# dhansmair/flamingo-mini

Measured on AMD Instinct MI355X. Metric: images/sec (fwd+bwd) flamingo-mini bs=32, higher is better.
Workload: dtype bf16

## Files before the change

flamingo-mini_amd/csrc/ff_api.hip:

```cpp
#include <stdarg.h>
#include <stdio.h>
#include <math.h>
#include <stdlib.h>
#include "ff_common.h"
#include "ff_internal.h"

namespace ff {

static thread_local char g_err[512] = "";
void set_error(const char* fmt, ...) {
    va_list ap;
    va_start(ap, fmt);
    vsnprintf(g_err, sizeof(g_err), fmt, ap);
    va_end(ap);
}
#ifdef FF_DEBUG
int dbg_switch(const char* name, int dflt) {
    const char* e = getenv(name);
    return e ? atoi(e) : dflt;
}
#endif
int check_launch(const char* what) {
    hipError_t e = hipGetLastError();
    if (e != hipSuccess) {
// ... 464 lines not shown
    return align_up(a.used);
}
struct XaScratch {
    void *dy1, *dH, *dxn, *dO, *dQs, *dKV, *dyn, *ws;
    size_t ws_bytes;
    float* lnx;
};
struct XaStash {
    void *dy1, *dH, *dQs;
    float *lnp_f = nullptr, *lnp_a = nullptr;
};
static bool xa_ln_deferrable(const XaDims& s) {
    static const int on = dbg_switch("FF_DEFER_LN", 1);
    return on != 0 && layernorm_bwd_deferrable(s.dt, s.d);
}
static size_t xa_stash_layout(const XaDims& s, void* base, size_t cap, XaStash& o) {
    Arena a(base, cap);
    const size_t M = (size_t)s.b * s.L;
    o.dy1 = a.take(M * s.d * s.es);
    o.dH = a.take(M * s.ffi * s.es);
    o.dQs = a.take(M * s.inner * s.es);
    if (xa_ln_deferrable(s)) {
        o.lnp_f = a.take<float>(layernorm_bwd_partial_bytes((int)M, s.d));
        o.lnp_a = a.take<float>(layernorm_bwd_partial_bytes((int)M, s.d));
    }
    return align_up(a.used);
}
static size_t xa_ws_bytes(const XaDims& s) {
    const int M = s.b * s.L, Mk = s.b * s.Nk;
    size_t w = 0;
    auto g = [&](int m, int n, int k) { w = std::max(w, gemm_workspace_bytes(s.dt, m, n, k, 1, 0)); };
    g(M, s.inner, s.d); g(Mk, 2 * s.inner, s.dv); g(M, s.d, s.inner); g(M, s.ffi, s.d); g(M, s.d, s.ffi);
    g(s.d, s.ffi, M); g(s.ffi, s.d, M); g(s.d, s.inner, M); g(s.inner, s.d, M); g(2 * s.inner, s.dv, Mk); g(Mk, s.dv, 2 * s.inner);
    w = std::max(w, layernorm_bwd_workspace(M, s.d));
    w = std::max(w, gate_grad_workspace(M, s.d));
    if (decode_ffw_supported(s.dt, M, s.d, s.ffi)) w = std::max(w, decode_ffw_workspace_bytes(s.d, s.ffi));
    return align_up(w) + align_up((size_t)s.b * s.H * s.L * 4);
}
// ... 32 lines not shown
    a.q = sq; a.o = sq; a.dq = sq; a.dout = sq;
    a.k = cached ? x.cached_k : sk;
    a.v = cached ? x.cached_v : sk;
    a.dk = sk; a.dv = sk;
    return a;
}

static bool xa_fused_enabled() {
    static const int v = dbg_switch("FF_XATTN_FUSED", 1);
    return v != 0;
}
static bool xa_ln3_enabled() {
    static const int v = dbg_switch("FF_XATTN_LN3", 1);
    return v != 0;
}
static XaFusedArgs xa_fused_args(const ff_xattn_desc& x, const XaDims& s, bool ext_kv) {
    XaFusedArgs a = {};
    a.batch = s.b; a.heads = s.H; a.n_q = s.L; a.n_kv = s.Nk; a.n_visual = s.nv; a.tt_stride = x.tt_stride; a.tt_offset = x.tt_offset;
    a.dim = s.d; a.inner = s.inner; a.scale = s.scale; a.eps = 1e-5f;
    static const int xcd_split = dbg_switch("FF_XATTN_XCD_SPLIT", 0);
    a.xcd_split = xcd_split;
    const ff_strides sk = {(long long)s.Nk * 2 * s.inner, 2LL * s.inner, s.dh};
    a.k = ext_kv ? x.cached_k : sk;
    a.v = ext_kv ? x.cached_v : sk;
    a.dk = sk; a.dv = sk;
    return a;
}

static bool xa_ln3_in_bwd(const ff_xattn_desc& x, const XaDims& s) {
    if (!xa_ln3_enabled() || !xa_fused_enabled() || !xa_fused_supported(s.dt, s.dh, s.d, s.inner) || x.sync == nullptr) return false;
    const XaFusedArgs fa = xa_fused_args(x, s, s.ext_kv);
    const int M = s.b * s.L;
    return xa_out_fusable(fa, s.dt, s.dh) && s.b <= layernorm_bwd_partial_blocks(M) && (size_t)s.b * (2 * (size_t)s.d + 2) * sizeof(float) <= layernorm_bwd_workspace(M, s.d);
}
static int xattn_fwd(const ff_xattn_desc* d, const void* y, const void* vf, const int* tt, const void* const* P, const void* ck,
                     const void* cv, void* y_out, void* saved, size_t saved_bytes, void* scratch, size_t scratch_bytes, hipStream_t st) {
    FF_TRY(xa_check(d));
    const bool cached = ck != nullptr;
    FF_CHECK(y && tt && P && y_out && saved && scratch && (cached ? cv != nullptr : vf != nullptr), FF_ERR_SHAPE, "xattn_fwd: null argument");
    const XaDims s(*d);
    FF_CHECK(s.ext_kv == cached, FF_ERR_SHAPE, "xattn_fwd: external K / V need their strides in the descriptor (cached_k / cached_v) and vice versa");
    XaSaved S;
    XaScratch W;
    FF_CHECK(xa_saved_layout(s, saved, saved_bytes, S) <= saved_bytes, FF_ERR_WORKSPACE, "xattn_fwd: saved buffer too small");
    FF_CHECK(xa_scratch_layout(s, scratch, scratch_bytes, false, W) <= scratch_bytes, FF_ERR_WORKSPACE, "xattn_fwd: scratch too small");
    const int M = s.b * s.L, Mk = s.b * s.Nk;
    const RowMap pd = plain_rows(s.d), pI = plain_rows(s.inner), pF = plain_rows(s.ffi), pV = plain_rows(s.dv), pKV = plain_rows(2 * s.inner);
    const void *Kp, *Vp;
    if (!cached) {
// ... 32 lines not shown
                     const void* saved, size_t saved_bytes, void* const* G, void* dy, void* dvf, void* scratch, size_t scratch_bytes,
                     hipStream_t st, const void* ext_k = nullptr, const void* ext_v = nullptr, void* dkv_out = nullptr,
                     void* stash = nullptr, size_t stash_bytes = 0) {
    FF_TRY(xa_check(d));
    const bool hoisted = ext_k != nullptr;
    FF_CHECK(y && tt && P && dy2 && saved && G && dy && scratch && (hoisted ? (ext_v && dkv_out) : vf != nullptr), FF_ERR_SHAPE,
             "xattn_bwd: null argument");
    const XaDims s(*d);
    FF_CHECK(s.ext_kv == hoisted, FF_ERR_SHAPE, "xattn_bwd: external K / V need their strides in the descriptor (cached_k / cached_v) and vice versa");
    XaSaved S;
    XaScratch W;
    FF_CHECK(xa_saved_layout(s, (void*)saved, saved_bytes, S) <= saved_bytes, FF_ERR_WORKSPACE, "xattn_bwd: saved buffer too small");
    FF_CHECK(xa_scratch_layout(s, scratch, scratch_bytes, true, W) <= scratch_bytes, FF_ERR_WORKSPACE, "xattn_bwd: scratch too small");
    XaStash T{W.dy1, W.dH, W.dQs};
    const bool defer = stash != nullptr;
    if (defer) FF_CHECK(xa_stash_layout(s, stash, stash_bytes, T) <= stash_bytes, FF_ERR_WORKSPACE, "xattn_bwd: stash too small");
    const bool defer_ln = defer && xa_ln_deferrable(s);
    if (defer_ln)
        FF_CHECK(((uintptr_t)y | (uintptr_t)dy | (uintptr_t)dy2 | (uintptr_t)P[2] | (uintptr_t)P[7]) % 16 == 0, FF_ERR_SHAPE,
                 "xattn_bwd (deferred weight gradients): y, d y_out, d y and the LayerNorm weights must be 16-byte aligned");
    LnPending pend_f, pend_a;
    const int M = s.b * s.L, Mk = s.b * s.Nk;
    const RowMap pd = plain_rows(s.d), pI = plain_rows(s.inner), pF = plain_rows(s.ffi), pV = plain_rows(s.dv), pKV = plain_rows(2 * s.inner);
    const size_t attn_ws_bytes = align_up((size_t)s.b * s.H * s.L * 4);
    const size_t gws = W.ws_bytes - attn_ws_bytes;
    float* attn_ws = (float*)((char*)W.ws + gws);

    if (!defer) FF_TRY(Gemm(s.dt, s.d, s.ffi, M).a(1, pd).b(1, pF).c(pF).problem(dy2, S.Aact, G[10], nullptr, nullptr, nullptr, P[1]).run(W.ws, gws, st));
    FF_TRY(Gemm(s.dt, M, s.ffi, s.d).a(0, pd).b(1, pF).c(pF).act_bwd(s.act).problem(dy2, P[10], T.dH, nullptr, S.Hpre, nullptr, P[1]).run(W.ws, gws, st));
    if (!defer) FF_TRY(Gemm(s.dt, s.ffi, s.d, M).a(1, pF).b(1, pd).c(pd).problem(T.dH, S.xn_f, G[9]).run(W.ws, gws, st));
    static const int fold_reduce = dbg_switch("FF_FOLD_SPLITK_LN", 1);
    int dxn_splits = 1;
    FF_TRY(Gemm(s.dt, M, s.d, s.ffi).a(0, pF).b(1, pd).c(pd).problem(T.dH, P[9], W.dxn).run(W.ws, gws, st, defer_ln && fold_reduce ? &dxn_splits : nullptr));
    {
        LnDots dots;
        dots.a = S.ffw_out; dots.alpha_a = P[1]; dots.out_a = G[1];
        dots.b = S.attn_out; dots.alpha_b = P[0]; dots.out_b = G[0];
        if (defer_ln) {
            LnArgs la = ln_args(s.dt, M, s.d, pd, pd, pd);
            if (dxn_splits > 1) { la.dy_splits = dxn_splits; la.dy_slab = (long long)M * s.d; }
            FF_TRY(layernorm_bwd(la, dxn_splits > 1 ? W.ws : W.dxn, S.y1, nullptr, P[7], S.mean_f, S.rstd_f, T.dy1, dy2, G[7], G[8], T.lnp_f,
                                 layernorm_bwd_partial_bytes(M, s.d), st, &dots, &pend_f));
            FF_CHECK(pend_f.partial, FF_ERR_SHAPE, "xattn_bwd: the one-pass LayerNorm backward did not apply in the deferred mode");
        } else FF_TRY(layernorm_bwd(ln_args(s.dt, M, s.d, pd, pd, pd), W.dxn, S.y1, nullptr, P[7], S.mean_f, S.rstd_f, T.dy1, dy2, G[7], G[8], W.ws, gws, st, &dots));
    }
    if (!defer) FF_TRY(Gemm(s.dt, s.d, s.inner, M).a(1, pd).b(1, pI).c(pI).problem(T.dy1, S.O, G[6], nullptr, nullptr, nullptr, P[0]).run(W.ws, gws, st));
    char* dK = hoisted ? (char*)dkv_out : (char*)W.dKV;
    char* dV = dK + (size_t)s.inner * s.es;
    const void* Kp = hoisted ? ext_k : S.KV;
    const void* Vp = hoisted ? ext_v : (const void*)((const char*)S.KV + (size_t)s.inner * s.es);
    bool dyn_fused = false, lnb_fused = false;
    float* lnb_partial = nullptr;
    if (xa_fused_enabled() && xa_fused_supported(s.dt, s.dh, s.d, s.inner)) {
        int single = 0;
        const XaFusedArgs fa = xa_fused_args(*d, s, hoisted);
        XaOutArgs oa = {(const bf16*)P[4], nullptr, (bf16*)W.dyn, nullptr, (unsigned*)d->sync};
        dyn_fused = d->sync != nullptr && xa_out_fusable(fa, s.dt, s.dh);
        if (dyn_fused && xa_ln3_in_bwd(*d, s)) {
            lnb_fused = true;
            lnb_partial = defer_ln ? T.lnp_a : (float*)W.ws;
            oa.out = nullptr;
            oa.ln_g = (const bf16*)P[2]; oa.ln_x = (const bf16*)y; oa.ln_res = (const bf16*)T.dy1; oa.ln_out = (bf16*)dy;
            oa.ln_mean = S.mean_a; oa.ln_rstd = S.rstd_a; oa.ln_part = W.lnx; oa.ln_wpart = lnb_partial;
        }
        FF_TRY(xa_dattn_bwd(fa, s.dt, s.dh, T.dy1, P[6], P[0], S.Qs, Kp, Vp, tt, S.O, S.lse, W.dO, T.dQs, dK, dV, attn_ws, &single, st,
                            dyn_fused ? &oa : nullptr));
        if (!single) FF_TRY(attention_bwd_dkv(xa_attn_desc(*d, s, hoisted), S.Qs, Kp, Vp, tt, W.dO, S.lse, attn_ws, dK, dV, st));
        if (lnb_fused && !defer_ln) {
            LnPending q;
            q.partial = lnb_partial; q.nblk = s.b; q.cols = s.d; q.dgamma = G[2]; q.dbeta = G[3];
            FF_TRY(layernorm_bwd_finish(s.dt, &q, 1, st));
        }
    } else {
        FF_TRY(Gemm(s.dt, M, s.inner, s.d).a(0, pd).b(1, pI).c(pI).problem(T.dy1, P[6], W.dO, nullptr, nullptr, nullptr, P[0]).run(W.ws, gws, st));
        FF_TRY(attention_bwd(xa_attn_desc(*d, s, hoisted), S.Qs, Kp, Vp, tt, S.O, W.dO, S.lse, T.dQs, dK, dV, attn_ws, (size_t)s.b * s.H * s.L * 4, st));
    }
    if (!defer) FF_TRY(Gemm(s.dt, s.inner, s.d, M).a(1, pI).b(1, pd).c(pd).scale(s.scale).problem(T.dQs, S.yn, G[4]).run(W.ws, gws, st));
    if (!hoisted) {
        FF_TRY(Gemm(s.dt, 2 * s.inner, s.dv, Mk).a(1, pKV).b(1, pV).c(pV).problem(W.dKV, vf, G[5]).run(W.ws, gws, st));
        if (dvf) FF_TRY(Gemm(s.dt, Mk, s.dv, 2 * s.inner).a(0, pKV).b(1, pV).c(pV).problem(W.dKV, P[5], dvf).run(W.ws, gws, st));
    }
// ... 26 lines not shown
    const int M = s.b * s.L;
    const RowMap pd = plain_rows(s.d), pI = plain_rows(s.inner), pF = plain_rows(s.ffi);
    LnPending ln_sets[2 * kGemmMaxZ];
    const bool finish_ln = xa_ln_deferrable(s);
    const int ln_blocks = layernorm_bwd_partial_blocks(M);
    Gemm g3(s.dt, s.d, s.ffi, M), g1(s.dt, s.ffi, s.d, M), go(s.dt, s.d, s.inner, M), gq(s.dt, s.inner, s.d, M);
    g3.a(1, pd).b(1, pF).c(pF);
    g1.a(1, pF).b(1, pd).c(pd);
    go.a(1, pd).b(1, pI).c(pI);
    gq.a(1, pI).b(1, pd).c(pd).scale(s.scale);
    for (int i = 0; i < n; i++) {
        XaSaved S;
        XaStash T;
        FF_CHECK(dy2[i] && saved[i] && stash[i], FF_ERR_SHAPE, "xattn_wgrad_grouped: null buffer of block %d", i);
        FF_CHECK(xa_saved_layout(s, (void*)saved[i], saved_bytes, S) <= saved_bytes, FF_ERR_WORKSPACE, "xattn_wgrad_grouped: saved buffer too small");
        FF_CHECK(xa_stash_layout(s, (void*)stash[i], stash_bytes, T) <= stash_bytes, FF_ERR_WORKSPACE, "xattn_wgrad_grouped: stash too small");
        const void* const* P = params + (size_t)i * FF_XATTN_PARAMS;
        void* const* G = grads + (size_t)i * FF_XATTN_PARAMS;
        FF_CHECK(G[10] && G[9] && G[6] && G[4] && P[0] && P[1], FF_ERR_SHAPE, "xattn_wgrad_grouped: null parameter / gradient of block %d", i);
        g3.problem(dy2[i], S.Aact, G[10], nullptr, nullptr, nullptr, P[1]);
        g1.problem(T.dH, S.xn_f, G[9]);
        go.problem(T.dy1, S.O, G[6], nullptr, nullptr, nullptr, P[0]);
        gq.problem(T.dQs, S.yn, G[4]);
        if (finish_ln) {
            FF_CHECK(G[0] && G[1] && G[2] && G[3] && G[7] && G[8], FF_ERR_SHAPE, "xattn_wgrad_grouped: null LayerNorm / gate gradient of block %d", i);
            LnPending& f = ln_sets[2 * i];
            f.partial = T.lnp_f; f.nblk = ln_blocks; f.cols = s.d; f.dgamma = G[7]; f.dbeta = G[8];
            f.alpha_a = P[1]; f.out_a = G[1]; f.alpha_b = P[0]; f.out_b = G[0];
            LnPending& q = ln_sets[2 * i + 1];
            q.partial = T.lnp_a; q.nblk = xa_ln3_in_bwd(*d, s) ? s.b : ln_blocks; q.cols = s.d; q.dgamma = G[2]; q.dbeta = G[3];
        }
    }
    if (finish_ln) FF_TRY(layernorm_bwd_finish(s.dt, ln_sets, 2 * n, st));
    FF_TRY(g3.run(ws, ws_bytes, st));
    FF_TRY(g1.run(ws, ws_bytes, st));
    FF_TRY(go.run(ws, ws_bytes, st));
    return gq.run(ws, ws_bytes, st);
}

static int kvp_check(const ff_kvproj_desc* d) {
    FF_CHECK(d, FF_ERR_SHAPE, "kv_project: null descriptor");
    FF_CHECK(d->dtype == FF_DTYPE_F32 || d->dtype == FF_DTYPE_BF16, FF_ERR_UNSUPPORTED, "kv_project: dtype %d", d->dtype);
// ... 171 lines not shown
    return ff::xattn_bwd(d, y, visual_features, text_time, params, dy_out, saved, saved_bytes, grads, dy, dvisual_features, scratch,
                         scratch_bytes, (hipStream_t)stream);
}

extern "C" int ff_xattn_block_bwd_kv(const ff_xattn_desc* d, const void* y, const void* k, const void* v, const int* text_time,
                                     const void* const* params, const void* dy_out, const void* saved, size_t saved_bytes,
                                     void* const* grads, void* dy, void* dkv, void* scratch, size_t scratch_bytes, ff_stream_t stream) {
    using namespace ff;
    FF_CHECK(k && v && dkv, FF_ERR_SHAPE, "ff_xattn_block_bwd_kv: null K / V / dKV");
    return xattn_bwd(d, y, nullptr, text_time, params, dy_out, saved, saved_bytes, grads, dy, nullptr, scratch, scratch_bytes,
                     (hipStream_t)stream, k, v, dkv);
}
extern "C" size_t ff_xattn_wgrad_stash_bytes(const ff_xattn_desc* d) {
    if (ff::xa_check(d) != FF_OK) return 0;
    ff::XaStash T;
    return ff::xa_stash_layout(ff::XaDims(*d), nullptr, 0, T);
}
extern "C" size_t ff_xattn_wgrad_workspace_bytes(const ff_xattn_desc* d) {
    if (ff::xa_check(d) != FF_OK) return 0;
    return ff::xa_wgrad_ws_bytes(ff::XaDims(*d));
}
extern "C" int ff_xattn_block_bwd_kv_data(const ff_xattn_desc* d, const void* y, const void* k, const void* v, const int* text_time,
                                          const void* const* params, const void* dy_out, const void* saved, size_t saved_bytes,
                                          void* const* grads, void* dy, void* dkv, void* stash, size_t stash_bytes, void* scratch,
                                          size_t scratch_bytes, ff_stream_t stream) {
    using namespace ff;
    FF_CHECK(k && v && dkv && stash, FF_ERR_SHAPE, "ff_xattn_block_bwd_kv_data: null K / V / dKV / stash");
    return xattn_bwd(d, y, nullptr, text_time, params, dy_out, saved, saved_bytes, grads, dy, nullptr, scratch, scratch_bytes,
                     (hipStream_t)stream, k, v, dkv, stash, stash_bytes);
}
extern "C" int ff_xattn_wgrad_grouped(const ff_xattn_desc* d, int n_blocks, const void* const* dy_out, const void* const* saved,
// ... 18 lines not shown
```

flamingo-mini_amd/csrc/ff_internal.h:

```cpp
#pragma once
#include <algorithm>
#include "ff_common.h"

namespace ff {

constexpr int kGemmMaxZ = 12;
constexpr int kKvProjGroup = 4;
struct GemmProblem {
    const void* A;
    const void* B;
    void* C;
    void* aux_out;
    const void* aux_in;
    const void* residual;
    const void* gate;
};
struct GemmParams {
    int M, N, K;
    int a_layout, b_layout;
    RowMap a_map, b_map, c_map, r_map;
    float scale;
    int act, act_bwd;
    int split_k, k_per_split;
    int tile;
// ... 99 lines not shown
    const bf16* W;
    const bf16* gate;
    bf16* out;
    bf16* aux;
    unsigned* sync;
    const bf16* ln_g;
    const bf16* ln_b;
    bf16* ln_out;
    float* ln_mean;
    float* ln_rstd;
    const bf16* ln_x;
    const bf16* ln_res;
    float* ln_part;
    float* ln_wpart;
};
size_t xa_ln3_part_bytes(int batch, int heads);
bool xa_out_fusable(const XaFusedArgs& a, int dtype, int dim_head);
bool xa_fused_supported(int dtype, int dim_head, int dim, int inner);
int xa_qattn_fwd(const XaFusedArgs& a, int dtype, int dim_head, const void* y, const void* gamma, const void* beta, const void* Wq, const void* K,
                 const void* V, const int* tt, void* yn, void* Qs, void* O, float* mean, float* rstd, float* lse, hipStream_t st,
                 const XaOutArgs* out = nullptr);
int xa_dattn_bwd(const XaFusedArgs& a, int dtype, int dim_head, const void* dy1, const void* Wo, const void* gate, const void* Qs, const void* K,
                 const void* V, const int* tt, const void* O, const float* lse, void* dO, void* dQ, void* dK, void* dV, float* Dsum,
                 int* single_tile, hipStream_t st, const XaOutArgs* out = nullptr);

bool decode_ffw_supported(int dtype, int M, int d, int ffi);
size_t decode_ffw_workspace_bytes(int d, int ffi);
int decode_ffw(int M, int d, int ffi, int act, float eps, const void* y1, const void* gamma, const void* beta, const void* W1, const void* W3,
               const void* alpha, void* xn, float* mean, float* rstd, void* Hpre, void* Aact, void* ffw_out, void* y_out, void* ws, size_t ws_bytes,
               hipStream_t st);

struct Arena {
    unsigned char* base;
    size_t cap, used;
    Arena(void* p, size_t c) : base((unsigned char*)p), cap(c), used(0) {}
    template <typename T = void> T* take(size_t bytes) {
        size_t at = align_up(used);
        used = at + bytes;
        return (T*)(base ? base + at : nullptr);
// ... 6 lines not shown
```

flamingo-mini_amd/csrc/ff_xattn_fused.hip:

```cpp
#include <atomic>
#include "ff_common.h"
#include "ff_internal.h"
#include "ff_gemm_tiles.h"
#include "ff_attention_core.h"

namespace ff {

#ifdef FF_XA_TIMELINE
__device__ unsigned long long g_xa_timeline[4096 * 16];
#define FF_XTL(i) do { if (threadIdx.x == 0 && blockIdx.x < 4096) g_xa_timeline[blockIdx.x * 16 + (i)] = __builtin_amdgcn_s_memrealtime(); } while (0)
#else
#define FF_XTL(i) do { } while (0)
#endif

namespace {

template <typename T> struct IsBf16 { static constexpr bool value = false; };
template <> struct IsBf16<bf16> { static constexpr bool value = true; };

template <typename T, int DH> struct Fast { static constexpr bool value = IsBf16<T>::value && DH == 64; };

struct DmaStage64 {
    typedef SwzLayout L;
    static FF_DEV void issue(bf16* s, const bf16* base, long long sr, int row0, int n_rows) {
// ... 762 lines not shown
                           ((unsigned long long)__builtin_bit_cast(unsigned, vb) << 32) | (unsigned long long)__builtin_bit_cast(unsigned, va), __ATOMIC_RELAXED,
                           __HIP_MEMORY_SCOPE_AGENT);
    asm volatile("s_waitcnt vmcnt(0)" ::: "memory");
    res_barrier();
    if (t == 0) res_await(cnt, res_arrive(cnt, (unsigned)heads), status);
    res_barrier();
    if (t < n_rows * heads) {
        const int r = t / heads, hh = t - r * heads;
        const unsigned long long v = __hip_atomic_load(granule + ((long long)(b * heads + hh) * 32 + r), __ATOMIC_RELAXED, __HIP_MEMORY_SCOPE_AGENT);
        stat[t * 2] = __builtin_bit_cast(float, (unsigned)(v & 0xffffffffull));
        stat[t * 2 + 1] = __builtin_bit_cast(float, (unsigned)(v >> 32));
    }
    __syncthreads();
}

}

template <int NSB, bool OUTP>
__global__ __launch_bounds__(512) void xa_qattn_fwd_res_kernel(const XaFusedArgs a_in, const bf16* __restrict__ y, const bf16* __restrict__ gamma,
                                                               const bf16* __restrict__ beta, const bf16* __restrict__ Wq, const bf16* __restrict__ K,
                                                               const bf16* __restrict__ V, const int* __restrict__ tt, bf16* __restrict__ yn,
                                                               bf16* __restrict__ Qs, bf16* O, float* __restrict__ mean,
                                                               float* __restrict__ rstd, float* __restrict__ lse, const XaOutArgs o_in) {
    extern __shared__ __attribute__((aligned(16))) unsigned char smem[];
    FF_XTL(0);
    const XaFusedArgs a = fetch_args(a_in);
    constexpr int DH = kResDH, BM = kResBM, NT = DH / 16;
    int h, b;
    res_work_item(a, h, b);
    const int t = threadIdx.x, l = t & 63, c = l & 15, g = l >> 4;
// ... 254 lines not shown
        if (i < n_items) {
            const int r = i / cpr, c8 = i - r * cpr;
            const float mean = L3.fin[2 * r], rs = L3.fin[2 * r + 1];
            float gv[8], bv[8], xn[8];
            unpack16(greg[u], gv, bf16());
            unpack16(breg[u], bv, bf16());
#pragma unroll
            for (int e = 0; e < 8; e++) xn[e] = (y1r[u][e] - mean) * rs * gv[e] + bv[e];
            Vec<bf16>::store(oa.ln_out + ((long long)b * a.n_q + r) * a.dim + n0 + c8 * 8, xn);
        }
    }
    FF_XTL(9);
}

template <int NSB, bool OUTP>
__global__ __launch_bounds__(512) void xa_dattn_bwd_res_kernel(const XaFusedArgs a_in, const bf16* __restrict__ dy1, const bf16* __restrict__ Wo,
                                                               const bf16* __restrict__ gate, const bf16* __restrict__ Qs, const bf16* __restrict__ K,
                                                               const bf16* __restrict__ V, const int* __restrict__ tt, const bf16* __restrict__ O,
                                                               const float* __restrict__ lse, bf16* dQ, bf16* __restrict__ dK,
                                                               bf16* __restrict__ dV, float* __restrict__ Dsum, const XaOutArgs o_in) {
    extern __shared__ __attribute__((aligned(16))) unsigned char smem[];
    FF_XTL(0);
    const XaFusedArgs a = fetch_args(a_in);
    constexpr int DH = kResDH, BM = kResBM, NT = DH / 16;
    typedef SwzLayout L;
    int h, b;
    res_work_item(a, h, b);
    const int t = threadIdx.x, l = t & 63, c = l & 15, g = l >> 4;
    const int w = __builtin_amdgcn_readfirstlane(t >> 6);
    const int nk = a.dim / kBK, n_rows = a.n_q;
    bf16* sA = (bf16*)smem;
    bf16* sB = sA + nk * (BM * kBK);
    bf16* sQ = sB + NSB * (DH * kBK);
    bf16* sK = sQ + L::tile_elems;
    bf16* sV = sK + L::tile_elems;
// ... 3 lines not shown
    int* s_flag = s_hi + kTile;
    float* s_lse = (float*)(s_flag + kTile);
    float* s_D = s_lse + kTile;
    bf16* sDO = sB;

    const int m_own = (w & 3) * 16 + c;
    const bool att = w < 4;
    const bool own_ok = att && m_own < n_rows;
    const ff_attn_desc d = attn_view(a, DH);
    const RowRange rr_full = row_range(d, tt, b, own_ok ? m_own : a.n_q);
    RowRange rr = rr_full;
    if (!own_ok || !rr.softmax) rr.lo = rr.hi = 0;
    const long long sidx = ((long long)b * a.heads + h) * a.n_q + m_own;
    const float Lq = own_ok ? lse[sidx] : kPosBig;
    if (t < kTile) { s_lo[t] = 0; s_hi[t] = 0; s_flag[t] = 0; s_lse[t] = kPosBig; s_D[t] = 0.f; }
    res_issue_rows(dy1 + (long long)b * a.n_q * a.dim, a.dim, n_rows, sA, w, l);
    const bf16* Kb = K + b * a.k.sb + h * a.k.sh;
    const bf16* Vb = V + b * a.v.sb + h * a.v.sh;
    const bf16* Qb = Qs + (long long)b * a.n_q * a.inner + h * DH;
    const bf16* Ob = O + (long long)b * a.n_q * a.inner + h * DH;
    {
        const int which = w >> 1;
        const bf16* src = which == 0 ? Qb : which == 1 ? Kb : which == 2 ? Vb : Ob;
        bf16* dst = which == 0 ? sQ : which == 1 ? sK : which == 2 ? sV : sO;
        const long long sr = which == 0 || which == 3 ? (long long)a.inner : which == 1 ? a.k.sr : a.v.sr;
        const int lim = which == 0 || which == 3 ? a.n_q : a.n_kv;
        const __amdgpu_buffer_rsrc_t rt = __builtin_amdgcn_make_buffer_rsrc((void*)src, 0, 0x7fffffff, 0x00020000);
        dma_tile<64, 0, 2>(rt, dst, RowMap{sr, 0, 0}, 0, lim, 0, kBK, w & 1, l);
    }
    const __amdgpu_buffer_rsrc_t rw = __builtin_amdgcn_make_buffer_rsrc((void*)Wo, 0, 0x7fffffff, 0x00020000);
    const RowMap w_map{a.inner, 0, 0};
    unsigned vb[2] = {kOobOffset, kOobOffset};
    if (w >= 4) {
        res_ring_start<NSB, 1>(rw, sB, w_map, h * DH, (h + 1) * DH, nk, w - 4, l, vb);
        wait_vmcnt<2 * (NSB - 1)>();
    } else wait_vmcnt<0>();
    res_barrier();
    FF_XTL(1);

    f32x4 acc[2] = {f32x4{0.f, 0.f, 0.f, 0.f}, f32x4{0.f, 0.f, 0.f, 0.f}};
    res_project<NSB, 1>(sA, sB, rw, w_map, vb, nk, w, acc);
    __syncthreads();
    FF_XTL(2);
    const float gt = tanhf(to_f32(gate[0]));
    if (w < 4) res_park(sDO, acc, gt, w, c, g);
    else {
        const int row = 32 + (w - 4) * 8 + (l >> 3), ch = l & 7;
        *(uint4*)(sDO + row * 64 + ch * 8) = uint4{0, 0, 0, 0};
    }
    __syncthreads();

// ... 57 lines not shown
    res_barrier();
    if (t == 0) res_await(cnt, target, oa.sync + kSyncStatus);
    res_barrier();
    FF_XTL(5);
    bf16* sA2 = sB;
    res_issue_rows_sc1(dQ + (long long)b * a.n_q * a.inner, a.inner, n_rows, sA2, w, l);
    wait_vmcnt<0>();
    res_barrier();
    FF_XTL(6);
    float* sP = (float*)ring2;
    const bool ln3 = oa.ln_out != nullptr;
    const int cpr = cs / 8, ld = cs + 4, n_items = n_rows * cpr;
    uint4 xreg[2] = {uint4{0, 0, 0, 0}, uint4{0, 0, 0, 0}}, greg[2] = {uint4{0, 0, 0, 0}, uint4{0, 0, 0, 0}}, rreg[2] = {uint4{0, 0, 0, 0}, uint4{0, 0, 0, 0}};
    float mu_r[2] = {0.f, 0.f}, rs_r[2] = {0.f, 0.f};
    if (ln3) {
#pragma unroll
        for (int u = 0; u < 2; u++) {
            const int i = t + u * 512;
            if (i < n_items) {
                const int r = i / cpr, c8 = i - r * cpr;
                const long long go = ((long long)b * a.n_q + r) * a.dim + n0 + c8 * 8;
                xreg[u] = *(const uint4*)(oa.ln_x + go);
                rreg[u] = *(const uint4*)(oa.ln_res + go);
                greg[u] = *(const uint4*)(oa.ln_g + n0 + c8 * 8);
                mu_r[u] = oa.ln_mean[(long long)b * a.n_q + r];
                rs_r[u] = oa.ln_rstd[(long long)b * a.n_q + r];
            }
        }
    }
    FF_RES_PER(per, (res_out_phase<PER, 1>(sA2, ring2, rwq, vo, wq_step, nk2, w, c, g, sP)));
    __syncthreads();
    FF_XTL(7);
    float dyh[2][8], xh[2][8];
    const Ln3Smem L3 = ln3_smem((float*)sB);
    const int cld = cs + 1;
#pragma unroll
    for (int u = 0; u < 2; u++) {
        const int i = t + u * 512;
// ... 125 lines not shown
        if (nk >= nsb && (bwd ? res_lds_bwd(a.dim, nsb) : res_lds_fwd(a.dim, nsb)) <= 160 * 1024) return nsb;
    return 0;
}
template <int NSB, bool OUTP>
static int launch_fwd_res(const XaFusedArgs& a, const void* y, const void* gamma, const void* beta, const void* Wq, const void* K, const void* V,
                          const int* tt, void* yn, void* Qs, void* O, float* mean, float* rstd, float* lse, const XaOutArgs& out, hipStream_t st) {
    const size_t lds = res_lds_fwd(a.dim, NSB);
    auto kernel = xa_qattn_fwd_res_kernel<NSB, OUTP>;
    FF_TRY(allow_lds(kernel, lds, "xa_qattn_fwd_res"));
    kernel<<<dim3(a.heads * a.batch), dim3(512), lds, st>>>(a, (const bf16*)y, (const bf16*)gamma, (const bf16*)beta, (const bf16*)Wq, (const bf16*)K,
                                                             (const bf16*)V, tt, (bf16*)yn, (bf16*)Qs, (bf16*)O, mean, rstd, lse, out);
    return check_launch("xa_qattn_fwd_res");
}
template <int NSB, bool OUTP>
static int launch_bwd_res(const XaFusedArgs& a, const void* dy1, const void* Wo, const void* gate, const void* Qs, const void* K, const void* V,
                          const int* tt, const void* O, const float* lse, void* dQ, void* dK, void* dV, float* Dsum, const XaOutArgs& out, hipStream_t st) {
    const size_t lds = res_lds_bwd(a.dim, NSB);
    auto kernel = xa_dattn_bwd_res_kernel<NSB, OUTP>;
    FF_TRY(allow_lds(kernel, lds, "xa_dattn_bwd_res"));
    kernel<<<dim3(a.heads * a.batch), dim3(512), lds, st>>>(a, (const bf16*)dy1, (const bf16*)Wo, (const bf16*)gate, (const bf16*)Qs, (const bf16*)K,
                                                             (const bf16*)V, tt, (const bf16*)O, lse, (bf16*)dQ, (bf16*)dK, (bf16*)dV, Dsum, out);
    return check_launch("xa_dattn_bwd_res");
}

size_t xa_ln3_part_bytes(int batch, int heads) { return (size_t)batch * heads * 32 * 2 * sizeof(float); }
constexpr int kMinCusPerXcd = 16;
static bool xa_exchange_device_ok() {
    static std::atomic<int> cache[64];
    int dev = 0;
    if (hipGetDevice(&dev) != hipSuccess || dev < 0 || dev >= 64) return false;
    int c = cache[dev].load(std::memory_order_relaxed);
    if (c == 0) {
        int cus = 0, xccs = 0;
        const bool have = hipDeviceGetAttribute(&cus, hipDeviceAttributeMultiprocessorCount, dev) == hipSuccess &&
                          hipDeviceGetAttribute(&xccs, hipDeviceAttributeNumberOfXccs, dev) == hipSuccess;
        c = (have && xccs == 8 && cus / 8 >= kMinCusPerXcd) ? 1 : 2;
// ... 32 lines not shown

template <typename T, int DH, int BM, bool SINGLE>
static int launch_bwd(const XaFusedArgs& a, const void* dy1, const void* Wo, const void* gate, const void* Qs, const void* K, const void* V,
                      const int* tt, const void* O, const float* lse, void* dO, void* dQ, void* dK, void* dV, float* Dsum, hipStream_t st) {
    const size_t lds = bwd_lds<T, DH, BM>();
    auto kernel = xa_dattn_bwd_kernel<T, DH, BM, SINGLE>;
    FF_TRY(allow_lds(kernel, lds, "xa_dattn_bwd"));
    const dim3 grid(cdiv(a.n_q, BM) * a.heads * a.batch);
    kernel<<<grid, dim3(256), lds, st>>>(a, (const T*)dy1, (const T*)Wo, (const T*)gate, (const T*)Qs, (const T*)K, (const T*)V, tt, (const T*)O, lse,
                                         (T*)dO, (T*)dQ, (T*)dK, (T*)dV, Dsum);
    return check_launch("xa_dattn_bwd");
}

int xa_dattn_bwd(const XaFusedArgs& a, int dtype, int dim_head, const void* dy1, const void* Wo, const void* gate, const void* Qs, const void* K,
                 const void* V, const int* tt, const void* O, const float* lse, void* dO, void* dQ, void* dK, void* dV, float* Dsum,
                 int* single_tile, hipStream_t st, const XaOutArgs* out) {
    FF_CHECK(xa_fused_supported(dtype, dim_head, a.dim, a.inner), FF_ERR_UNSUPPORTED, "xa_dattn_bwd: unsupported dtype / head size");
    FF_CHECK(dy1 && Wo && gate && Qs && K && V && tt && O && lse && dQ && dK && dV && Dsum && single_tile, FF_ERR_SHAPE, "xa_dattn_bwd: null argument");
    FF_CHECK(!out || (xa_out_fusable(a, dtype, dim_head) && out->W && (out->out || out->ln_out) && out->sync), FF_ERR_SHAPE,
             "xa_dattn_bwd: phase 2 (d LN(y) inside the launch) asked for a problem that does not take it, or with a null argument");
    FF_CHECK(!out || !out->ln_out || (out->ln_g && out->ln_x && out->ln_res && out->ln_mean && out->ln_rstd && out->ln_part && out->ln_wpart), FF_ERR_SHAPE,
             "xa_dattn_bwd: phase 3 (LayerNorm backward inside the launch) with a null argument");
    const bool single = a.n_q <= 64;
    FF_CHECK(single || dO, FF_ERR_SHAPE, "xa_dattn_bwd: dO buffer needed when the queries span several tiles");
    *single_tile = single ? 1 : 0;
    const int pid = profile_begin(dtype, out ? (out->ln_out ? -9 : -7) : -5, a.heads, 0, a.n_q, a.n_kv, a.dim, a.batch * a.heads, dim_head, st);
    int rc;
    const int nsb = res_ring_depth(a, dtype, dim_head, true);
    const XaOutArgs none = {};
    if (nsb == 6 && out) rc = launch_bwd_res<6, true>(a, dy1, Wo, gate, Qs, K, V, tt, O, lse, dQ, dK, dV, Dsum, *out, st);
    else if (nsb == 4 && out) rc = launch_bwd_res<4, true>(a, dy1, Wo, gate, Qs, K, V, tt, O, lse, dQ, dK, dV, Dsum, *out, st);
    else if (nsb == 6) rc = launch_bwd_res<6, false>(a, dy1, Wo, gate, Qs, K, V, tt, O, lse, dQ, dK, dV, Dsum, none, st);
    else if (nsb == 4) rc = launch_bwd_res<4, false>(a, dy1, Wo, gate, Qs, K, V, tt, O, lse, dQ, dK, dV, Dsum, none, st);
    else if (a.n_q <= 32) FF_XA_DISPATCH(dtype, dim_head, rc = (launch_bwd<T, DH, 32, true>(a, dy1, Wo, gate, Qs, K, V, tt, O, lse, dO, dQ, dK, dV, Dsum, st)));
    else if (single) FF_XA_DISPATCH(dtype, dim_head, rc = (launch_bwd<T, DH, 64, true>(a, dy1, Wo, gate, Qs, K, V, tt, O, lse, dO, dQ, dK, dV, Dsum, st)));
    else FF_XA_DISPATCH(dtype, dim_head, rc = (launch_bwd<T, DH, 64, false>(a, dy1, Wo, gate, Qs, K, V, tt, O, lse, dO, dQ, dK, dV, Dsum, st)));
    profile_end(pid, st);
    return rc;
}

}

#ifdef FF_XA_TIMELINE
extern "C" int ff_debug_xa_timeline_read(unsigned long long* out, int n_blocks) {
    return (int)hipMemcpyFromSymbol(out, HIP_SYMBOL(ff::g_xa_timeline), sizeof(unsigned long long) * 16 * n_blocks);
}
#endif
```

Baseline: 792.7.

## Fuse LayerNorm(y1) backward into the fused cross-attention backward kernel

Adds a phase 0 to the persistent cross-attention backward kernel. It reduces the split-K dxn partials, computes the LayerNorm(y1) input gradient plus residual, and writes gate dot products and per-head dgamma/dbeta partials. This replaces the separate layernorm_bwd launch before the attention backward. A grid-wide arrive/await then makes the dy1 rows visible before they are reloaded with sc1 loads. The cost is the extra in-kernel sync, more partial rows to reduce later (batch×heads), and a larger stash.

```diff
diff --git a/flamingo-mini_amd/csrc/ff_api.hip b/flamingo-mini_amd/csrc/ff_api.hip
--- a/flamingo-mini_amd/csrc/ff_api.hip
+++ b/flamingo-mini_amd/csrc/ff_api.hip
@@ -502,14 +502,17 @@
     static const int on = dbg_switch("FF_DEFER_LN", 1);
     return on != 0 && layernorm_bwd_deferrable(s.dt, s.d);
 }
-static size_t xa_stash_layout(const XaDims& s, void* base, size_t cap, XaStash& o) {
+static bool xa_ln0_shape(const ff_xattn_desc& x, const XaDims& s);
+static size_t xa_stash_layout(const ff_xattn_desc& x, const XaDims& s, void* base, size_t cap, XaStash& o) {
     Arena a(base, cap);
     const size_t M = (size_t)s.b * s.L;
     o.dy1 = a.take(M * s.d * s.es);
     o.dH = a.take(M * s.ffi * s.es);
     o.dQs = a.take(M * s.inner * s.es);
     if (xa_ln_deferrable(s)) {
-        o.lnp_f = a.take<float>(layernorm_bwd_partial_bytes((int)M, s.d));
+        size_t lnp_f = layernorm_bwd_partial_bytes((int)M, s.d);
+        if (xa_ln0_shape(x, s)) lnp_f = std::max(lnp_f, (size_t)s.b * s.H * (2 * (size_t)s.d + 2) * sizeof(float));
+        o.lnp_f = a.take<float>(lnp_f);
         o.lnp_a = a.take<float>(layernorm_bwd_partial_bytes((int)M, s.d));
     }
     return align_up(a.used);
@@ -572,6 +575,10 @@
     static const int v = dbg_switch("FF_XATTN_LN3", 1);
     return v != 0;
 }
+static bool xa_ln0_enabled() {
+    static const int v = dbg_switch("FF_XATTN_LN0", 1);
+    return v != 0;
+}
 static XaFusedArgs xa_fused_args(const ff_xattn_desc& x, const XaDims& s, bool ext_kv) {
     XaFusedArgs a = {};
     a.batch = s.b; a.heads = s.H; a.n_q = s.L; a.n_kv = s.Nk; a.n_visual = s.nv; a.tt_stride = x.tt_stride; a.tt_offset = x.tt_offset;
@@ -591,6 +598,11 @@
     const int M = s.b * s.L;
     return xa_out_fusable(fa, s.dt, s.dh) && s.b <= layernorm_bwd_partial_blocks(M) && (size_t)s.b * (2 * (size_t)s.d + 2) * sizeof(float) <= layernorm_bwd_workspace(M, s.d);
 }
+static bool xa_ln0_shape(const ff_xattn_desc& x, const XaDims& s) {
+    if (!xa_ln0_enabled() || !xa_fused_enabled() || !xa_fused_supported(s.dt, s.dh, s.d, s.inner) || !xa_ln_deferrable(s)) return false;
+    return xa_out_fusable(xa_fused_args(x, s, s.ext_kv), s.dt, s.dh);
+}
+static bool xa_ln0_in_bwd(const ff_xattn_desc& x, const XaDims& s) { return x.sync != nullptr && xa_ln0_shape(x, s); }
 static int xattn_fwd(const ff_xattn_desc* d, const void* y, const void* vf, const int* tt, const void* const* P, const void* ck,
                      const void* cv, void* y_out, void* saved, size_t saved_bytes, void* scratch, size_t scratch_bytes, hipStream_t st) {
     FF_TRY(xa_check(d));
@@ -653,7 +665,7 @@
     FF_CHECK(xa_scratch_layout(s, scratch, scratch_bytes, true, W) <= scratch_bytes, FF_ERR_WORKSPACE, "xattn_bwd: scratch too small");
     XaStash T{W.dy1, W.dH, W.dQs};
     const bool defer = stash != nullptr;
-    if (defer) FF_CHECK(xa_stash_layout(s, stash, stash_bytes, T) <= stash_bytes, FF_ERR_WORKSPACE, "xattn_bwd: stash too small");
+    if (defer) FF_CHECK(xa_stash_layout(*d, s, stash, stash_bytes, T) <= stash_bytes, FF_ERR_WORKSPACE, "xattn_bwd: stash too small");
     const bool defer_ln = defer && xa_ln_deferrable(s);
     if (defer_ln)
         FF_CHECK(((uintptr_t)y | (uintptr_t)dy | (uintptr_t)dy2 | (uintptr_t)P[2] | (uintptr_t)P[7]) % 16 == 0, FF_ERR_SHAPE,
@@ -670,12 +682,18 @@
     if (!defer) FF_TRY(Gemm(s.dt, s.ffi, s.d, M).a(1, pF).b(1, pd).c(pd).problem(T.dH, S.xn_f, G[9]).run(W.ws, gws, st));
     static const int fold_reduce = dbg_switch("FF_FOLD_SPLITK_LN", 1);
     int dxn_splits = 1;
+    const bool ln0 = defer_ln && xa_ln0_in_bwd(*d, s);
+    XaLn0Args l0 = {};
     FF_TRY(Gemm(s.dt, M, s.d, s.ffi).a(0, pF).b(1, pd).c(pd).problem(T.dH, P[9], W.dxn).run(W.ws, gws, st, defer_ln && fold_reduce ? &dxn_splits : nullptr));
     {
         LnDots dots;
         dots.a = S.ffw_out; dots.alpha_a = P[1]; dots.out_a = G[1];
         dots.b = S.attn_out; dots.alpha_b = P[0]; dots.out_b = G[0];
-        if (defer_ln) {
+        if (ln0) {
+            l0.dln = dxn_splits > 1 ? W.ws : W.dxn; l0.splits = dxn_splits > 1 ? dxn_splits : 0; l0.slab = (long long)M * s.d;
+            l0.x = (const bf16*)S.y1; l0.gamma = (const bf16*)P[7]; l0.mean = S.mean_f; l0.rstd = S.rstd_f; l0.res = (const bf16*)dy2;
+            l0.dot_a = (const bf16*)S.ffw_out; l0.dot_b = (const bf16*)S.attn_out; l0.dx = (bf16*)T.dy1; l0.part = T.lnp_f;
+        } else if (defer_ln) {
             LnArgs la = ln_args(s.dt, M, s.d, pd, pd, pd);
             if (dxn_splits > 1) { la.dy_splits = dxn_splits; la.dy_slab = (long long)M * s.d; }
             FF_TRY(layernorm_bwd(la, dxn_splits > 1 ? W.ws : W.dxn, S.y1, nullptr, P[7], S.mean_f, S.rstd_f, T.dy1, dy2, G[7], G[8], T.lnp_f,
@@ -695,6 +713,7 @@
         const XaFusedArgs fa = xa_fused_args(*d, s, hoisted);
         XaOutArgs oa = {(const bf16*)P[4], nullptr, (bf16*)W.dyn, nullptr, (unsigned*)d->sync};
         dyn_fused = d->sync != nullptr && xa_out_fusable(fa, s.dt, s.dh);
+        FF_CHECK(!ln0 || dyn_fused, FF_ERR_SHAPE, "xattn_bwd: LayerNorm(y1) backward was left to a launch that does not take it");
         if (dyn_fused && xa_ln3_in_bwd(*d, s)) {
             lnb_fused = true;
             lnb_partial = defer_ln ? T.lnp_a : (float*)W.ws;
@@ -703,7 +722,7 @@
             oa.ln_mean = S.mean_a; oa.ln_rstd = S.rstd_a; oa.ln_part = W.lnx; oa.ln_wpart = lnb_partial;
         }
         FF_TRY(xa_dattn_bwd(fa, s.dt, s.dh, T.dy1, P[6], P[0], S.Qs, Kp, Vp, tt, S.O, S.lse, W.dO, T.dQs, dK, dV, attn_ws, &single, st,
-                            dyn_fused ? &oa : nullptr));
+                            dyn_fused ? &oa : nullptr, ln0 ? &l0 : nullptr));
         if (!single) FF_TRY(attention_bwd_dkv(xa_attn_desc(*d, s, hoisted), S.Qs, Kp, Vp, tt, W.dO, S.lse, attn_ws, dK, dV, st));
         if (lnb_fused && !defer_ln) {
             LnPending q;
@@ -760,7 +779,7 @@
         XaStash T;
         FF_CHECK(dy2[i] && saved[i] && stash[i], FF_ERR_SHAPE, "xattn_wgrad_grouped: null buffer of block %d", i);
         FF_CHECK(xa_saved_layout(s, (void*)saved[i], saved_bytes, S) <= saved_bytes, FF_ERR_WORKSPACE, "xattn_wgrad_grouped: saved buffer too small");
-        FF_CHECK(xa_stash_layout(s, (void*)stash[i], stash_bytes, T) <= stash_bytes, FF_ERR_WORKSPACE, "xattn_wgrad_grouped: stash too small");
+        FF_CHECK(xa_stash_layout(*d, s, (void*)stash[i], stash_bytes, T) <= stash_bytes, FF_ERR_WORKSPACE, "xattn_wgrad_grouped: stash too small");
         const void* const* P = params + (size_t)i * FF_XATTN_PARAMS;
         void* const* G = grads + (size_t)i * FF_XATTN_PARAMS;
         FF_CHECK(G[10] && G[9] && G[6] && G[4] && P[0] && P[1], FF_ERR_SHAPE, "xattn_wgrad_grouped: null parameter / gradient of block %d", i);
@@ -771,7 +790,7 @@
         if (finish_ln) {
             FF_CHECK(G[0] && G[1] && G[2] && G[3] && G[7] && G[8], FF_ERR_SHAPE, "xattn_wgrad_grouped: null LayerNorm / gate gradient of block %d", i);
             LnPending& f = ln_sets[2 * i];
-            f.partial = T.lnp_f; f.nblk = ln_blocks; f.cols = s.d; f.dgamma = G[7]; f.dbeta = G[8];
+            f.partial = T.lnp_f; f.nblk = xa_ln0_in_bwd(*d, s) ? s.b * s.H : ln_blocks; f.cols = s.d; f.dgamma = G[7]; f.dbeta = G[8];
             f.alpha_a = P[1]; f.out_a = G[1]; f.alpha_b = P[0]; f.out_b = G[0];
             LnPending& q = ln_sets[2 * i + 1];
             q.partial = T.lnp_a; q.nblk = xa_ln3_in_bwd(*d, s) ? s.b : ln_blocks; q.cols = s.d; q.dgamma = G[2]; q.dbeta = G[3];
@@ -973,7 +992,7 @@
 extern "C" size_t ff_xattn_wgrad_stash_bytes(const ff_xattn_desc* d) {
     if (ff::xa_check(d) != FF_OK) return 0;
     ff::XaStash T;
-    return ff::xa_stash_layout(ff::XaDims(*d), nullptr, 0, T);
+    return ff::xa_stash_layout(*d, ff::XaDims(*d), nullptr, 0, T);
 }
 extern "C" size_t ff_xattn_wgrad_workspace_bytes(const ff_xattn_desc* d) {
     if (ff::xa_check(d) != FF_OK) return 0;
diff --git a/flamingo-mini_amd/csrc/ff_internal.h b/flamingo-mini_amd/csrc/ff_internal.h
--- a/flamingo-mini_amd/csrc/ff_internal.h
+++ b/flamingo-mini_amd/csrc/ff_internal.h
@@ -137,6 +137,20 @@
     float* ln_part;
     float* ln_wpart;
 };
+struct XaLn0Args {
+    const void* dln;
+    long long slab;
+    int splits, pad_;
+    const bf16* x;
+    const bf16* gamma;
+    const float* mean;
+    const float* rstd;
+    const bf16* res;
+    const bf16* dot_a;
+    const bf16* dot_b;
+    bf16* dx;
+    float* part;
+};
 size_t xa_ln3_part_bytes(int batch, int heads);
 bool xa_out_fusable(const XaFusedArgs& a, int dtype, int dim_head);
 bool xa_fused_supported(int dtype, int dim_head, int dim, int inner);
@@ -145,7 +159,7 @@
                  const XaOutArgs* out = nullptr);
 int xa_dattn_bwd(const XaFusedArgs& a, int dtype, int dim_head, const void* dy1, const void* Wo, const void* gate, const void* Qs, const void* K,
                  const void* V, const int* tt, const void* O, const float* lse, void* dO, void* dQ, void* dK, void* dV, float* Dsum,
-                 int* single_tile, hipStream_t st, const XaOutArgs* out = nullptr);
+                 int* single_tile, hipStream_t st, const XaOutArgs* out = nullptr, const XaLn0Args* ln0 = nullptr);
 
 bool decode_ffw_supported(int dtype, int M, int d, int ffi);
 size_t decode_ffw_workspace_bytes(int d, int ffi);
diff --git a/flamingo-mini_amd/csrc/ff_xattn_fused.hip b/flamingo-mini_amd/csrc/ff_xattn_fused.hip
--- a/flamingo-mini_amd/csrc/ff_xattn_fused.hip
+++ b/flamingo-mini_amd/csrc/ff_xattn_fused.hip
@@ -800,6 +800,142 @@
     __syncthreads();
 }
 
+FF_DEV void res_ln0_phase(const XaFusedArgs& a, const XaLn0Args& q, unsigned* cnt, unsigned* status, int b, int h, int n_rows, int t, int w, int l,
+                          float* simg) {
+    typedef __attribute__((ext_vector_type(4))) unsigned u32x4;
+    const int j = w >> 1, row = h + a.heads * j;
+    const bool own = row < n_rows;
+    const int pl = (w & 1) * 64 + l, nchunk = a.dim / 8;
+    const long long grow = (long long)b * a.n_q + row;
+    float* red = simg + 8 * a.dim;
+    float xh[2][8], dv[2][8];
+    uint4 gq[2], rq[2], ra[2], rb[2];
+    bool ok[2];
+    float s1 = 0.f, s2 = 0.f, da = 0.f, db = 0.f;
+    float mu = 0.f, rs = 0.f;
+    if (own) { mu = q.mean[grow]; rs = q.rstd[grow]; }
+    {
+        uint4 xq[2];
+#pragma unroll
+        for (int i = 0; i < 2; i++) {
+            const int c = pl + 128 * i;
+            ok[i] = own && c < nchunk;
+            xq[i] = gq[i] = rq[i] = ra[i] = rb[i] = uint4{0, 0, 0, 0};
+            if (ok[i]) {
+                const long long off = grow * a.dim + c * 8;
+                xq[i] = *(const uint4*)(q.x + off);
+                gq[i] = *(const uint4*)(q.gamma + c * 8);
+                rq[i] = *(const uint4*)(q.res + off);
+                ra[i] = *(const uint4*)(q.dot_a + off);
+                rb[i] = *(const uint4*)(q.dot_b + off);
+            }
+        }
+#pragma unroll
+        for (int i = 0; i < 2; i++) {
+#pragma unroll
+            for (int e = 0; e < 8; e++) dv[i][e] = 0.f;
+            if (!ok[i]) continue;
+            const long long off = grow * a.dim + (pl + 128 * i) * 8;
+            if (q.splits > 0) {
+                const float* pp = (const float*)q.dln + off;
+                for (int sp = 0; sp < q.splits; sp += 4) {
+                    f32x4 v[4][2];
+#pragma unroll
+                    for (int u = 0; u < 4; u++)
+                        if (sp + u < q.splits) {
+                            v[u][0] = *(const f32x4*)(pp + (long long)(sp + u) * q.slab);
+                            v[u][1] = *(const f32x4*)(pp + (long long)(sp + u) * q.slab + 4);
+                        }
+#pragma unroll
+                    for (int u = 0; u < 4; u++)
+                        if (sp + u < q.splits) {
+#pragma unroll
+                            for (int e = 0; e < 4; e++) { dv[i][e] += v[u][0][e]; dv[i][4 + e] += v[u][1][e]; }
+                        }
+                }
+            } else {
+                const uint4 dq = *(const uint4*)((const bf16*)q.dln + off);
+                unpack16(dq, dv[i], bf16());
+            }
+        }
+#pragma unroll
+        for (int i = 0; i < 2; i++) {
+            float xv[8], gv[8];
+            unpack16(xq[i], xv, bf16());
+            unpack16(gq[i], gv, bf16());
+#pragma unroll
+            for (int e = 0; e < 8; e++) {
+                const float dyh = dv[i][e] * gv[e];
+                xh[i][e] = ok[i] ? (xv[e] - mu) * rs : 0.f;
+                s1 += dyh;
+                s2 += dyh * xh[i][e];
+            }
+        }
+    }
+    s1 = wave_sum(s1);
+    s2 = wave_sum(s2);
+    if (l == 0) { red[w * 2] = s1; red[w * 2 + 1] = s2; }
+    res_barrier();
+    FF_XTL(12);
+    const float m1 = (red[(w & ~1) * 2] + red[(w | 1) * 2]) / (float)a.dim, m2 = (red[(w & ~1) * 2 + 1] + red[(w | 1) * 2 + 1]) / (float)a.dim;
+    const __amdgpu_buffer_rsrc_t rdx = __builtin_amdgcn_make_buffer_rsrc((void*)(q.dx + (long long)b * a.n_q * a.dim), 0, 0x7fffffff, 0x00020000);
+    float* img = simg + j * 2 * a.dim;
+#pragma unroll
+    for (int i = 0; i < 2; i++) {
+        const int c = pl + 128 * i;
+        if (c < nchunk) {
+            float gv[8], rv[8], ua[8], ub[8], o[8];
+            unpack16(gq[i], gv, bf16());
+            unpack16(rq[i], rv, bf16());
+            unpack16(ra[i], ua, bf16());
+            unpack16(rb[i], ub, bf16());
+#pragma unroll
+            for (int e = 0; e < 8; e++) {
+                o[e] = rs * (dv[i][e] * gv[e] - m1 - xh[i][e] * m2);
+                da += rv[e] * ua[e];
+                o[e] += rv[e];
+            }
+            bf16x8 ob;
+#pragma unroll
+            for (int e = 0; e < 8; e++) {
+                ob[e] = (bf16)o[e];
+                db += (float)ob[e] * ub[e];
+            }
+            if (ok[i]) __builtin_amdgcn_raw_buffer_store_b128(__builtin_bit_cast(u32x4, ob), rdx, (unsigned)(row * a.dim + c * 8) * 2u, 0, 16);
+#pragma unroll
+            for (int e = 0; e < 8; e += 4) {
+                *(f32x4*)(img + c * 8 + e) = f32x4{dv[i][e] * xh[i][e], dv[i][e + 1] * xh[i][e + 1], dv[i][e + 2] * xh[i][e + 2], dv[i][e + 3] * xh[i][e + 3]};
+                *(f32x4*)(img + a.dim + c * 8 + e) = f32x4{dv[i][e], dv[i][e + 1], dv[i][e + 2], dv[i][e + 3]};
+            }
+        }
+    }
+    da = wave_sum(da);
+    db = wave_sum(db);
+    if (l == 0) { red[16 + w * 2] = da; red[16 + w * 2 + 1] = db; }
+    asm volatile("s_waitcnt vmcnt(0)" ::: "memory");
+    res_barrier();
+    FF_XTL(13);
+    unsigned target = 0;
+    if (t == 0) target = res_arrive(cnt, (unsigned)a.heads);
+    float* out = q.part + (long long)(b * a.heads + h) * (2 * a.dim + 2);
+    for (int i = t * 4; i < 2 * a.dim; i += 512 * 4) {
+        const f32x4 v0 = *(const f32x4*)(simg + i), v1 = *(const f32x4*)(simg + 2 * a.dim + i);
+        const f32x4 v2 = *(const f32x4*)(simg + 4 * a.dim + i), v3 = *(const f32x4*)(simg + 6 * a.dim + i);
+        float* o = out + i;
+        o[0] = (v0[0] + v1[0]) + (v2[0] + v3[0]); o[1] = (v0[1] + v1[1]) + (v2[1] + v3[1]);
+        o[2] = (v0[2] + v1[2]) + (v2[2] + v3[2]); o[3] = (v0[3] + v1[3]) + (v2[3] + v3[3]);
+    }
+    if (t == 64) {
+        float sa = 0.f, sb = 0.f;
+        for (int u = 0; u < 8; u++) { sa += red[16 + u * 2]; sb += red[16 + u * 2 + 1]; }
+        out[2 * a.dim] = sa;
+        out[2 * a.dim + 1] = sb;
+    }
+    FF_XTL(14);
+    if (t == 0) res_await(cnt, target, status);
+    res_barrier();
+}
+
 }
 
 template <int NSB, bool OUTP>
@@ -1084,11 +1220,11 @@
 }
 
 template <int NSB, bool OUTP>
-__global__ __launch_bounds__(512) void xa_dattn_bwd_res_kernel(const XaFusedArgs a_in, const bf16* __restrict__ dy1, const bf16* __restrict__ Wo,
+__global__ __launch_bounds__(512) void xa_dattn_bwd_res_kernel(const XaFusedArgs a_in, const bf16* dy1, const bf16* __restrict__ Wo,
                                                                const bf16* __restrict__ gate, const bf16* __restrict__ Qs, const bf16* __restrict__ K,
                                                                const bf16* __restrict__ V, const int* __restrict__ tt, const bf16* __restrict__ O,
                                                                const float* __restrict__ lse, bf16* dQ, bf16* __restrict__ dK,
-                                                               bf16* __restrict__ dV, float* __restrict__ Dsum, const XaOutArgs o_in) {
+                                                               bf16* __restrict__ dV, float* __restrict__ Dsum, const XaOutArgs o_in, const XaLn0Args l0_in) {
     extern __shared__ __attribute__((aligned(16))) unsigned char smem[];
     FF_XTL(0);
     const XaFusedArgs a = fetch_args(a_in);
@@ -1122,7 +1258,8 @@
     const long long sidx = ((long long)b * a.heads + h) * a.n_q + m_own;
     const float Lq = own_ok ? lse[sidx] : kPosBig;
     if (t < kTile) { s_lo[t] = 0; s_hi[t] = 0; s_flag[t] = 0; s_lse[t] = kPosBig; s_D[t] = 0.f; }
-    res_issue_rows(dy1 + (long long)b * a.n_q * a.dim, a.dim, n_rows, sA, w, l);
+    const bool ln0 = OUTP && l0_in.dx != nullptr;
+    if (!ln0) res_issue_rows(dy1 + (long long)b * a.n_q * a.dim, a.dim, n_rows, sA, w, l);
     const bf16* Kb = K + b * a.k.sb + h * a.k.sh;
     const bf16* Vb = V + b * a.v.sb + h * a.v.sh;
     const bf16* Qb = Qs + (long long)b * a.n_q * a.inner + h * DH;
@@ -1139,10 +1276,15 @@
     const __amdgpu_buffer_rsrc_t rw = __builtin_amdgcn_make_buffer_rsrc((void*)Wo, 0, 0x7fffffff, 0x00020000);
     const RowMap w_map{a.inner, 0, 0};
     unsigned vb[2] = {kOobOffset, kOobOffset};
-    if (w >= 4) {
-        res_ring_start<NSB, 1>(rw, sB, w_map, h * DH, (h + 1) * DH, nk, w - 4, l, vb);
-        wait_vmcnt<2 * (NSB - 1)>();
-    } else wait_vmcnt<0>();
+    if (w >= 4) res_ring_start<NSB, 1>(rw, sB, w_map, h * DH, (h + 1) * DH, nk, w - 4, l, vb);
+    if (ln0) {
+        FF_XTL(10);
+        res_ln0_phase(a, l0_in, o_in.sync + kSyncSlots + (b % kSyncSlots), o_in.sync + kSyncStatus, b, h, n_rows, t, w, l, (float*)sA);
+        FF_XTL(11);
+        res_issue_rows_sc1(dy1 + (long long)b * a.n_q * a.dim, a.dim, n_rows, sA, w, l);
+        wait_vmcnt<0>();
+    } else if (w >= 4) wait_vmcnt<2 * (NSB - 1)>();
+    else wait_vmcnt<0>();
     res_barrier();
     FF_XTL(1);
 
@@ -1230,6 +1372,7 @@
     uint4 xreg[2] = {uint4{0, 0, 0, 0}, uint4{0, 0, 0, 0}}, greg[2] = {uint4{0, 0, 0, 0}, uint4{0, 0, 0, 0}}, rreg[2] = {uint4{0, 0, 0, 0}, uint4{0, 0, 0, 0}};
     float mu_r[2] = {0.f, 0.f}, rs_r[2] = {0.f, 0.f};
     if (ln3) {
+        const __amdgpu_buffer_rsrc_t rres = __builtin_amdgcn_make_buffer_rsrc((void*)(oa.ln_res + (long long)b * a.n_q * a.dim), 0, 0x7fffffff, 0x00020000);
 #pragma unroll
         for (int u = 0; u < 2; u++) {
             const int i = t + u * 512;
@@ -1237,7 +1380,9 @@
                 const int r = i / cpr, c8 = i - r * cpr;
                 const long long go = ((long long)b * a.n_q + r) * a.dim + n0 + c8 * 8;
                 xreg[u] = *(const uint4*)(oa.ln_x + go);
-                rreg[u] = *(const uint4*)(oa.ln_res + go);
+                if (ln0)
+                    rreg[u] = __builtin_bit_cast(uint4, __builtin_amdgcn_raw_buffer_load_b128(rres, (unsigned)(r * a.dim + n0 + c8 * 8) * 2u, 0, 16));
+                else rreg[u] = *(const uint4*)(oa.ln_res + go);
                 greg[u] = *(const uint4*)(oa.ln_g + n0 + c8 * 8);
                 mu_r[u] = oa.ln_mean[(long long)b * a.n_q + r];
                 rs_r[u] = oa.ln_rstd[(long long)b * a.n_q + r];
@@ -1393,12 +1538,12 @@
 }
 template <int NSB, bool OUTP>
 static int launch_bwd_res(const XaFusedArgs& a, const void* dy1, const void* Wo, const void* gate, const void* Qs, const void* K, const void* V,
-                          const int* tt, const void* O, const float* lse, void* dQ, void* dK, void* dV, float* Dsum, const XaOutArgs& out, hipStream_t st) {
+                          const int* tt, const void* O, const float* lse, void* dQ, void* dK, void* dV, float* Dsum, const XaOutArgs& out, const XaLn0Args& ln0, hipStream_t st) {
     const size_t lds = res_lds_bwd(a.dim, NSB);
     auto kernel = xa_dattn_bwd_res_kernel<NSB, OUTP>;
     FF_TRY(allow_lds(kernel, lds, "xa_dattn_bwd_res"));
     kernel<<<dim3(a.heads * a.batch), dim3(512), lds, st>>>(a, (const bf16*)dy1, (const bf16*)Wo, (const bf16*)gate, (const bf16*)Qs, (const bf16*)K,
-                                                             (const bf16*)V, tt, (const bf16*)O, lse, (bf16*)dQ, (bf16*)dK, (bf16*)dV, Dsum, out);
+                                                             (const bf16*)V, tt, (const bf16*)O, lse, (bf16*)dQ, (bf16*)dK, (bf16*)dV, Dsum, out, ln0);
     return check_launch("xa_dattn_bwd_res");
 }
 
@@ -1461,24 +1606,28 @@
 
 int xa_dattn_bwd(const XaFusedArgs& a, int dtype, int dim_head, const void* dy1, const void* Wo, const void* gate, const void* Qs, const void* K,
                  const void* V, const int* tt, const void* O, const float* lse, void* dO, void* dQ, void* dK, void* dV, float* Dsum,
-                 int* single_tile, hipStream_t st, const XaOutArgs* out) {
+                 int* single_tile, hipStream_t st, const XaOutArgs* out, const XaLn0Args* ln0) {
     FF_CHECK(xa_fused_supported(dtype, dim_head, a.dim, a.inner), FF_ERR_UNSUPPORTED, "xa_dattn_bwd: unsupported dtype / head size");
     FF_CHECK(dy1 && Wo && gate && Qs && K && V && tt && O && lse && dQ && dK && dV && Dsum && single_tile, FF_ERR_SHAPE, "xa_dattn_bwd: null argument");
     FF_CHECK(!out || (xa_out_fusable(a, dtype, dim_head) && out->W && (out->out || out->ln_out) && out->sync), FF_ERR_SHAPE,
              "xa_dattn_bwd: phase 2 (d LN(y) inside the launch) asked for a problem that does not take it, or with a null argument");
     FF_CHECK(!out || !out->ln_out || (out->ln_g && out->ln_x && out->ln_res && out->ln_mean && out->ln_rstd && out->ln_part && out->ln_wpart), FF_ERR_SHAPE,
              "xa_dattn_bwd: phase 3 (LayerNorm backward inside the launch) with a null argument");
+    FF_CHECK(!ln0 || (out && ln0->dln && ln0->x && ln0->gamma && ln0->mean && ln0->rstd && ln0->res && ln0->dot_a && ln0->dot_b && ln0->part && ln0->dx == dy1 &&
+                      ln0->splits >= 0),
+             FF_ERR_SHAPE, "xa_dattn_bwd: phase 0 (LayerNorm(y1) backward inside the launch) needs phase 2, every operand, and d y1 as its output");
     const bool single = a.n_q <= 64;
     FF_CHECK(single || dO, FF_ERR_SHAPE, "xa_dattn_bwd: dO buffer needed when the queries span several tiles");
     *single_tile = single ? 1 : 0;
-    const int pid = profile_begin(dtype, out ? (out->ln_out ? -9 : -7) : -5, a.heads, 0, a.n_q, a.n_kv, a.dim, a.batch * a.heads, dim_head, st);
+    const int pid = profile_begin(dtype, out ? (out->ln_out ? -9 : -7) : -5, a.heads, ln0 ? 1 : 0, a.n_q, a.n_kv, a.dim, a.batch * a.heads, dim_head, st);
     int rc;
     const int nsb = res_ring_depth(a, dtype, dim_head, true);
     const XaOutArgs none = {};
-    if (nsb == 6 && out) rc = launch_bwd_res<6, true>(a, dy1, Wo, gate, Qs, K, V, tt, O, lse, dQ, dK, dV, Dsum, *out, st);
-    else if (nsb == 4 && out) rc = launch_bwd_res<4, true>(a, dy1, Wo, gate, Qs, K, V, tt, O, lse, dQ, dK, dV, Dsum, *out, st);
-    else if (nsb == 6) rc = launch_bwd_res<6, false>(a, dy1, Wo, gate, Qs, K, V, tt, O, lse, dQ, dK, dV, Dsum, none, st);
-    else if (nsb == 4) rc = launch_bwd_res<4, false>(a, dy1, Wo, gate, Qs, K, V, tt, O, lse, dQ, dK, dV, Dsum, none, st);
+    const XaLn0Args no_ln0 = {};
+    if (nsb == 6 && out) rc = launch_bwd_res<6, true>(a, dy1, Wo, gate, Qs, K, V, tt, O, lse, dQ, dK, dV, Dsum, *out, ln0 ? *ln0 : no_ln0, st);
+    else if (nsb == 4 && out) rc = launch_bwd_res<4, true>(a, dy1, Wo, gate, Qs, K, V, tt, O, lse, dQ, dK, dV, Dsum, *out, ln0 ? *ln0 : no_ln0, st);
+    else if (nsb == 6) rc = launch_bwd_res<6, false>(a, dy1, Wo, gate, Qs, K, V, tt, O, lse, dQ, dK, dV, Dsum, none, no_ln0, st);
+    else if (nsb == 4) rc = launch_bwd_res<4, false>(a, dy1, Wo, gate, Qs, K, V, tt, O, lse, dQ, dK, dV, Dsum, none, no_ln0, st);
     else if (a.n_q <= 32) FF_XA_DISPATCH(dtype, dim_head, rc = (launch_bwd<T, DH, 32, true>(a, dy1, Wo, gate, Qs, K, V, tt, O, lse, dO, dQ, dK, dV, Dsum, st)));
     else if (single) FF_XA_DISPATCH(dtype, dim_head, rc = (launch_bwd<T, DH, 64, true>(a, dy1, Wo, gate, Qs, K, V, tt, O, lse, dO, dQ, dK, dV, Dsum, st)));
     else FF_XA_DISPATCH(dtype, dim_head, rc = (launch_bwd<T, DH, 64, false>(a, dy1, Wo, gate, Qs, K, V, tt, O, lse, dO, dQ, dK, dV, Dsum, st)));
```

New measurement: 794.7, median of 6. No clear change (+0.3%).
